# goldbricklemon/uplift-upsample-3dhpe

Hardware: AMD Instinct MI355X
Metric: pose-sequences/sec (higher is better)
Workload: dtype f16x3 (f32 operands split into f16 hi/lo, 3 MFMA passes, f32 accumulate); 1 GPU; config/h36m_351.json forward, N=71 tokens (receptive field 351), J=17, batch 128/GPU, s_in=5, seeded Keras-default weights; global_batch=128, parallelism=batch-sharded x1, hipgraph=True, concurrent_half_batches=False, batches_in_flight=8

## Files before the change

uplift-upsample-3dhpe_amd/csrc/uu3d_tchain16.h:

```cpp
#pragma once
#include <algorithm>
#include "uu3d_gemm_panel8.h"

namespace uu3d {

enum : int {
    TC_PROJ = 1,
    TC_MLP = 2,
    TC_QKV = 4,
    TC_FC1_PLANES = 8,
    TC_PE = 16,
};

static constexpr int TC_CHUNK_HALFS = P8_CHUNK_BYTES / 2;
__host__ __device__ inline constexpr int tchain_chunks(int flags) {
    return ((flags & TC_PROJ) ? 12 : 0) + ((flags & TC_MLP) ? 48 : 0) + ((flags & TC_FC1_PLANES) ? 24 : 0) + ((flags & TC_QKV) ? 36 : 0);
}
static constexpr size_t TC_TRASH_BYTES = 16384;

enum : int { TCP_BP = 0, TCP_B1 = 384, TCP_B2 = 1152, TCP_BQKV = 1536, TCP_FLOATS = 2688 };

struct TChainArgs {
    int M, m_tiles, period; float qscale;
    const _Float16* Of;
    float* X;
    float* XA; const float* pe;
    const _Float16* W;
    const float* P;
    _Float16* Q;
    _Float16* H;
    unsigned char* scratch;
};

__host__ __device__ inline size_t tchain_qf_index(size_t token, int ch, int plane) {
    const int u = ch >> 4, w = ch & 15, j = ((w >> 3) << 2) | (w & 3), g = (w >> 2) & 1;
    return ((((token >> 5) * 72 + u) * 2 + plane) * 64 + (token & 31) + 32 * g) * 8 + j;
}
__host__ __device__ inline constexpr size_t tchain_qf_halfs(int m_tiles) { return (size_t)m_tiles * 4 * 72 * 2 * 512; }

static constexpr size_t T16_X_FLOATS_PER_TILE = 64 * 384;
__host__ __device__ inline constexpr size_t tchain16_scratch_bytes(int m_tiles64) {
    return (size_t)m_tiles64 * (2 * T16_X_FLOATS_PER_TILE * 4) + TC_TRASH_BYTES;
}
inline void tchain16_reorder_mlp(const _Float16* in, _Float16* out) {
    const size_t C = TC_CHUNK_HALFS;
    std::copy(in, in + 12 * C, out);
    std::copy(in + 24 * C, in + 36 * C, out + 12 * C);
    std::copy(in + 12 * C, in + 24 * C, out + 24 * C);
    std::copy(in + 36 * C, in + 48 * C, out + 36 * C);
}

static constexpr size_t T16_XCHG_BYTES = 8 * 1024;
static constexpr size_t T16_BIAS_BYTES = 1152 * 4;
static constexpr size_t T16_LDS_TOTAL = P8_RING_BYTES + T16_XCHG_BYTES + T16_BIAS_BYTES;

__host__ __device__ inline size_t tchain16_xs_index(int row, int ch) {
    const int tile = row >> 6, q = (row >> 4) & 3, t = row & 15;
    const int c = ch >> 5, hh = (ch >> 4) & 1, g = (ch >> 2) & 3, r = ch & 3;
    return (size_t)tile * T16_X_FLOATS_PER_TILE + (((size_t)(c * 8 + 4 * hh + q) * 64 + t + 16 * g) * 4 + r);
}

inline void tchain16_pack_stage(const _Float16* Bh, const _Float16* Bl, int N, int Kp, int kofs, bool natural, _Float16* out) {
    for (int c = 0; c < N / 32; ++c)
        for (int hh = 0; hh < 2; ++hh)
            for (int kk = 0; kk < 12; ++kk)
                for (int p = 0; p < 2; ++p)
                    for (int l = 0; l < 64; ++l)
                        for (int j = 0; j < 8; ++j) {
                            const int S = kk >> 1, mm = kk & 1, t = l & 15, g = l >> 4;
                            const int n = 32 * c + 16 * (mm ^ hh) + t;
                            const int k = natural ? 16 * (12 * hh + 2 * S + (g >> 1)) + 8 * (j >> 2) + 4 * (g & 1) + (j & 3)
                                                  : kofs + 32 * (2 * S + (j >> 2)) + 16 * hh + 4 * g + (j & 3);
                            out[(((((size_t)c * 2 + hh) * 12 + kk) * 2 + p) * 64 + l) * 8 + j] = (p ? Bl : Bh)[(size_t)n * Kp + k];
                        }
}

template <bool BIAS> struct T16EpResidual { static constexpr int kStores = 0; static constexpr bool kBias = BIAS; const float* bias; int nbias; };
struct T16EpHidden { static constexpr int kStores = 0; static constexpr bool kBias = true; const float* bias; int nbias; };
struct T16EpQkv { static constexpr int kStores = 2; static constexpr bool kBias = true; h16x4* __restrict__ qf; const float* bias; int nbias; };
struct T16EpPlanes { static constexpr int kStores = 2; static constexpr bool kBias = true; unsigned char* __restrict__ ph; unsigned char* __restrict__ pl; const float* bias; int nbias; };

#ifndef UU3D_T16_DEPTH
#define UU3D_T16_DEPTH 2
#endif
#ifndef UU3D_T16_LOO
#define UU3D_T16_LOO 0
#endif

template <int FLAGS>
__global__ void __launch_bounds__(512) __attribute__((amdgpu_waves_per_eu(2, 2)))
tchain16_kernel(const TChainArgs a)
{
    constexpr int HS = 12, KS = 6;
    constexpr int GT = tchain_chunks(FLAGS);
    static_assert(!((FLAGS & TC_MLP) && (FLAGS & TC_FC1_PLANES)), "one MLP form per launch");
    static_assert(GT >= 12, "at least one stage");
    h3_flush_f16_denormals();
    extern __shared__ __attribute__((aligned(16))) unsigned char psm[];

    const int bm = blockIdx.x;
    const int tid = threadIdx.x, lane = tid & 63, wave = __builtin_amdgcn_readfirstlane(tid >> 6);
    const int hh = wave >> 2, q = wave & 3, g = lane >> 4, t = lane & 15;
    const int tok = bm * 64 + q * 16 + t;
    const bool live = tok < a.M;
    const int tokc = min(tok, a.M - 1);
    const int chl = 16 * hh + 4 * g;

    const unsigned wofs = (unsigned)(hh * HS * 2048 + q * 3072);
    const unsigned char* const wsrc = reinterpret_cast<const unsigned char*>(a.W) + wofs;
    const unsigned lane16 = (unsigned)lane * 16u;
    auto dma1 = [&](int Gc, int j, int slot, int i) __attribute__((always_inline)) {
        if (UU3D_T16_LOO & 1) return;
        const unsigned char* s = wsrc + (size_t)min(Gc, GT - 1) * P8_CHUNK_BYTES + j * (6 * 2048);
        unsigned char* d = psm + slot * P8_CHUNK_BYTES + wofs + j * (6 * 2048);
        switch (i) {
            case 0: __builtin_amdgcn_global_load_lds((h3_glb_void*)(s + lane16), (h3_lds_void*)d, 16, 0, 0); break;
            case 1: __builtin_amdgcn_global_load_lds((h3_glb_void*)(s + lane16), (h3_lds_void*)d, 16, 1024, 0); break;
            default: __builtin_amdgcn_global_load_lds((h3_glb_void*)(s + lane16), (h3_lds_void*)d, 16, 2048, 0); break;
        }
    };

    f32x4 xr[12];
    h16x8 ah[KS], al[KS];
    h16x8 fh[KS], fl[KS];
    constexpr int DP = UU3D_T16_DEPTH, RB = DP + 1;
    h16x8 bh[RB] = {}, bl[RB] = {};

    auto late = [&](int v) __attribute__((always_inline)) -> int { asm volatile("" : "+s"(v)); return v; };
    const unsigned xoff = (unsigned)(wave * 256 + lane * 4);
    auto xs_tile = [&](int b, bool strided1) __attribute__((always_inline)) -> float* {
        return reinterpret_cast<float*>(a.scratch) + ((size_t)b + (strided1 ? (size_t)a.m_tiles : 0)) * T16_X_FLOATS_PER_TILE;
    };
    auto load_xs = [&](const float* tl) __attribute__((always_inline)) {
#pragma unroll
        for (int c = 0; c < 12; ++c) xr[c] = *reinterpret_cast<const f32x4*>(tl + (xoff + (unsigned)(c * 2048)));
    };
    auto store_xs = [&](float* tl) __attribute__((always_inline)) {
        unsigned xo = xoff;
        asm volatile("" : "+v"(xo));
#pragma unroll
        for (int c = 0; c < 12; ++c) *reinterpret_cast<f32x4*>(tl + (xo + (unsigned)(c * 2048))) = xr[c];
    };
    auto load_rows = [&](const float* base) __attribute__((always_inline)) {
        const float* p = base + (size_t)tokc * 384 + chl;
#pragma unroll
        for (int c = 0; c < 12; ++c) xr[c] = *reinterpret_cast<const f32x4*>(p + 32 * c);
    };
    auto store_rows = [&](float* base) __attribute__((always_inline)) {
        const int tk = late(bm) * 64 + q * 16 + t;
        unsigned char* const tr = a.scratch + (size_t)a.m_tiles * (2 * T16_X_FLOATS_PER_TILE * 4);
        float* p = tk < a.M ? base + (size_t)tk * 384 + chl : reinterpret_cast<float*>(tr) + chl;
#pragma unroll
        for (int c = 0; c < 12; ++c) *reinterpret_cast<f32x4*>(p + 32 * c) = xr[c];
    };

    constexpr bool kStrided1 = (FLAGS & TC_FC1_PLANES) != 0;
    if constexpr ((FLAGS & TC_PROJ) != 0) {
        load_xs(xs_tile(bm, kStrided1));
        const int row0 = min(bm * 64 + q * 16, a.M - 1);
        const h16x8* ap = reinterpret_cast<const h16x8*>(a.Of) + (size_t)(row0 >> 5) * 24 * 2 * 64 + (row0 & 16) + t + 32 * (g & 1);
#pragma unroll
        for (int S = 0; S < KS; ++S) {
            const int sl = 12 * hh + 2 * S + (g >> 1);
            ah[S] = ap[(sl * 2 + 0) * 64]; al[S] = ap[(sl * 2 + 1) * 64];
        }
    } else {
        load_rows(a.X);
    }
#pragma unroll
    for (int g2 = 0; g2 < 5; ++g2)
#pragma unroll
        for (int i = 0; i < 3; ++i) dma1(g2 >> 1, g2 & 1, g2 >> 1, i);
    int G = 0, slot = 0;

    unsigned char* const xmine = psm + P8_RING_BYTES + wave * 1024 + lane16;
    unsigned char* const xpart = psm + P8_RING_BYTES + (wave ^ 4) * 1024 + lane16;
    float* const stat = reinterpret_cast<float*>(psm + P8_RING_BYTES);
    float* const bias_lds = reinterpret_cast<float*>(psm + P8_RING_BYTES + T16_XCHG_BYTES);
    const unsigned rd0 = (unsigned)(uintptr_t)(h3_lds_void*)(psm + hh * HS * 2048 + lane16);
    const unsigned bias_rd = (unsigned)(uintptr_t)(h3_lds_void*)(psm + P8_RING_BYTES + T16_XCHG_BYTES) + (unsigned)chl * 4u;

#define UU3D_T16_READ(i, sb, kk) \
    asm volatile("ds_read_b128 %0, %2 offset:%3\n\tds_read_b128 %1, %2 offset:%4" \
                 : "=&v"(bh[i]), "=&v"(bl[i]) : "v"(sb), "i"((kk) * 2048), "i"((kk) * 2048 + 1024))

    struct Acc { f32x4 a0[2], a1[2]; };
    struct Fin { f32x4 u, s, r, b, y; h16x4 vh, vl; };
    struct Keep { h16x4 h, l; };
    using I0 = std::integral_constant<int, 0>; using I1 = std::integral_constant<int, 1>; using I2 = std::integral_constant<int, 2>; using I3 = std::integral_constant<int, 3>;

    auto fin_a = [&](auto ep, auto fin_tag, const int j, Fin& f) __attribute__((always_inline)) {
        using EP = decltype(ep);
        constexpr int fs = decltype(fin_tag)::value;
        float y = f.u[j] + f.r[j];
        if constexpr (EP::kBias) y += f.b[j];
        if constexpr (std::is_same<EP, T16EpResidual<false>>::value || std::is_same<EP, T16EpResidual<true>>::value) {
            xr[fs][j] += y;
        } else {
            if constexpr (std::is_same<EP, T16EpHidden>::value || std::is_same<EP, T16EpPlanes>::value) y = fmaxf(y, 0.f);
            _Float16 h; float hf;
            asm("v_cvt_f16_f32 %0, %2\n\tv_cvt_f32_f16 %1, %0" : "=&v"(h), "=v"(hf) : "v"(y));
            f.y[j] = y - hf;
            f.vh[j] = h;
        }
    };
    auto fin_b = [&](auto ep, const int j, Fin& f) __attribute__((always_inline)) {
        using EP = decltype(ep);
        if constexpr (!(std::is_same<EP, T16EpResidual<false>>::value || std::is_same<EP, T16EpResidual<true>>::value))
            f.vl[j] = (_Float16)(f.y[j] * H3_SCALE);
    };
    auto fin_store = [&](auto ep, const int cp, auto fin_tag, Fin& f, Keep& hk) __attribute__((always_inline)) {
        using EP = decltype(ep);
        constexpr int fs = decltype(fin_tag)::value;
        if constexpr (std::is_same<EP, T16EpHidden>::value) {
            if constexpr ((fs & 1) == 0) { hk.h = f.vh; hk.l = f.vl; }
            else {
                h16x8 ph, pl;
#pragma unroll
                for (int e = 0; e < 4; ++e) { ph[e] = hk.h[e]; ph[4 + e] = f.vh[e]; pl[e] = hk.l[e]; pl[4 + e] = f.vl[e]; }
                constexpr int ks = fs == 11 ? 5 : fs >> 1;
                fh[ks] = ph; fl[ks] = pl;
            }
        } else if constexpr (std::is_same<EP, T16EpQkv>::value) {
            h16x4* d = ep.qf + (size_t)(2 * cp + hh) * 256;
            d[0] = f.vh; d[128] = f.vl;
        } else if constexpr (std::is_same<EP, T16EpPlanes>::value) {
            const unsigned o = (unsigned)(32 * cp) * 2u;
            *reinterpret_cast<h16x4*>(ep.ph + o) = f.vh;
            *reinterpret_cast<h16x4*>(ep.pl + o) = f.vl;
        }
    };

    auto chunk = [&](auto cl_tag, auto pre_tag, const int c, auto fin_tag, auto ep, const h16x8 (&Ah)[KS], const h16x8 (&Al)[KS],
                     Acc& x, const Acc& p, Keep& hk, const int bias_c0) __attribute__((always_inline)) {
        constexpr int CL = decltype(cl_tag)::value;
        constexpr bool PRE_IN = (decltype(pre_tag)::value & 1) != 0, PRE_OUT = (decltype(pre_tag)::value & 2) != 0;
        using EP = decltype(ep);
        constexpr int NST = EP::kStores;
        constexpr bool FIN = CL > 0 && !(UU3D_T16_LOO & 2);
        const int pslot = slot == 0 ? 2 : slot - 1;
        const unsigned sb = rd0 + (unsigned)slot * P8_CHUNK_BYTES;
        Fin f;
        auto gapwork = [&](const int gp) __attribute__((always_inline)) {
            if constexpr (CL > 0 && (UU3D_T16_LOO & 2) != 0) { if (gp == 3) asm volatile("" :: "v"(p.a0[0]), "v"(p.a0[1]), "v"(p.a1[0]), "v"(p.a1[1])); }
            if constexpr (FIN) {
                if (gp == 3 || gp == 4) {
#pragma unroll
                    for (int e = 0; e < 2; ++e) { const int k = 2 * (gp - 3) + e; f.s[k] = p.a0[1][k] + p.a1[1][k] * (1.0f / H3_SCALE); }
                }
                if (gp == 5) asm volatile("ds_write_b128 %0, %1" :: "v"((unsigned)(uintptr_t)(h3_lds_void*)xmine), "v"(f.s) : "memory");
                if (gp >= 9 && gp <= 12) f.u[gp - 9] = p.a0[0][gp - 9] + p.a1[0][gp - 9] * (1.0f / H3_SCALE);
                if (gp >= 22 && gp <= 25) fin_b(ep, gp - 22, f);
                if (gp >= 21 && gp <= 24) fin_a(ep, fin_tag, gp - 21, f);
                if (gp == 27) fin_store(ep, c - 1, fin_tag, f, hk);
            }
        };
        if constexpr (PRE_IN) asm volatile("s_waitcnt vmcnt(%0)" :: "i"(9 + NST * ((CL >= 2) + (CL >= 3))) : "memory");
        else asm volatile("s_waitcnt vmcnt(%0) lgkmcnt(0)" :: "i"(9 + NST * ((CL >= 2) + (CL >= 3))) : "memory");
        __builtin_amdgcn_sched_barrier(0);
        __builtin_amdgcn_s_barrier();
        __builtin_amdgcn_sched_barrier(0);
        if constexpr (!PRE_IN) {
#pragma unroll
            for (int d = 0; d < DP; ++d) UU3D_T16_READ(d, sb, d);
        }
#pragma unroll
        for (int m = 0; m < 2; ++m) { x.a0[m] = f32x4{0.f, 0.f, 0.f, 0.f}; x.a1[m] = f32x4{0.f, 0.f, 0.f, 0.f}; }
#define UU3D_T16_KK(kk) \
            x.a0[(kk) & 1] = __builtin_amdgcn_mfma_f32_16x16x32_f16(bh[(kk) % RB], Ah[(kk) >> 1], x.a0[(kk) & 1], 0, 0, 0); \
            __builtin_amdgcn_sched_barrier(0); gapwork(3 * (kk)); __builtin_amdgcn_sched_barrier(0); \
            x.a1[(kk) & 1] = __builtin_amdgcn_mfma_f32_16x16x32_f16(bh[(kk) % RB], Al[(kk) >> 1], x.a1[(kk) & 1], 0, 0, 0); \
            __builtin_amdgcn_sched_barrier(0); gapwork(3 * (kk) + 1); __builtin_amdgcn_sched_barrier(0); \
            x.a1[(kk) & 1] = __builtin_amdgcn_mfma_f32_16x16x32_f16(bl[(kk) % RB], Ah[(kk) >> 1], x.a1[(kk) & 1], 0, 0, 0); \
            __builtin_amdgcn_sched_barrier(0); gapwork(3 * (kk) + 2); __builtin_amdgcn_sched_barrier(0);
#pragma unroll
        for (int kk = 0; kk < 6; ++kk) {
            UU3D_T16_READ((kk + DP) % RB, sb, kk + DP);
            asm volatile("s_waitcnt lgkmcnt(%2)" : "+v"(bh[kk % RB]), "+v"(bl[kk % RB]) : "i"(2 * DP + (FIN && kk >= 2 && kk <= 1 + DP ? 1 : 0)));
            UU3D_T16_KK(kk)
            if ((kk & 1) == 0) dma1(G + 2, 1, pslot, kk >> 1);
            __builtin_amdgcn_sched_barrier(0);
        }
        asm volatile("s_waitcnt vmcnt(%0) lgkmcnt(%1)" :: "i"(9 + NST * (CL >= 2)), "i"(2 * DP) : "memory");
        __builtin_amdgcn_sched_barrier(0);
        __builtin_amdgcn_s_barrier();
        __builtin_amdgcn_sched_barrier(0);
        constexpr int NRB = FIN ? (EP::kBias ? 2 : 1) : 0;
        if constexpr (FIN) {
            asm volatile("ds_read_b128 %0, %1" : "=&v"(f.r) : "v"((unsigned)(uintptr_t)(h3_lds_void*)xpart) : "memory");
            if constexpr (EP::kBias) asm volatile("ds_read_b128 %0, %1" : "=&v"(f.b) : "v"(bias_rd + (unsigned)(bias_c0 + c - 1) * 128u) : "memory");
        }
#pragma unroll
        for (int kk = 6; kk < HS; ++kk) {
            if (kk + DP < HS) UU3D_T16_READ((kk + DP) % RB, sb, kk + DP);
            const int ahead = 2 * ((kk + DP < HS ? kk + DP : HS - 1) - kk);
            if (FIN && kk == 7) {
                const int behind = 6 + DP < HS ? 2 * ((7 + DP < HS ? 7 + DP : HS - 1) - (6 + DP) + 1) : 0;
                if constexpr (EP::kBias) asm volatile("s_waitcnt lgkmcnt(%4)" : "+v"(bh[kk % RB]), "+v"(bl[kk % RB]), "+v"(f.r), "+v"(f.b) : "i"(behind < ahead ? behind : ahead));
                else asm volatile("s_waitcnt lgkmcnt(%3)" : "+v"(bh[kk % RB]), "+v"(bl[kk % RB]), "+v"(f.r) : "i"(behind < ahead ? behind : ahead));
            }
            else asm volatile("s_waitcnt lgkmcnt(%2)" : "+v"(bh[kk % RB]), "+v"(bl[kk % RB]) : "i"(ahead + (FIN && kk == 6 ? NRB : 0)));
            UU3D_T16_KK(kk)
            if ((kk & 1) == 0) dma1(G + 3, 0, slot, (kk - 6) >> 1);
            __builtin_amdgcn_sched_barrier(0);
        }
#undef UU3D_T16_KK
        G += 1;
        slot = slot == 2 ? 0 : slot + 1;
        if constexpr (PRE_OUT) {
            const unsigned nb = rd0 + (unsigned)slot * P8_CHUNK_BYTES;
#pragma unroll
            for (int d = 0; d < DP; ++d) UU3D_T16_READ(d, nb, d);
        }
    };

    auto stage_tail = [&](auto ep, const int c, auto fin_tag, const Acc& p, Keep& hk, const int bias_c0) __attribute__((always_inline)) {
        using EP = decltype(ep);
        asm volatile("s_waitcnt vmcnt(0) lgkmcnt(0)" ::: "memory");
        __builtin_amdgcn_s_barrier();
        Fin f;
#pragma unroll
        for (int e = 0; e < 4; ++e) { f.s[e] = p.a0[1][e] + p.a1[1][e] * (1.0f / H3_SCALE); f.u[e] = p.a0[0][e] + p.a1[0][e] * (1.0f / H3_SCALE); }
        asm volatile("ds_write_b128 %0, %1\n\ts_waitcnt lgkmcnt(0)" :: "v"((unsigned)(uintptr_t)(h3_lds_void*)xmine), "v"(f.s) : "memory");
        __builtin_amdgcn_s_barrier();
        asm volatile("ds_read_b128 %0, %1" : "=&v"(f.r) : "v"((unsigned)(uintptr_t)(h3_lds_void*)xpart) : "memory");
        if constexpr (EP::kBias) asm volatile("ds_read_b128 %0, %1" : "=&v"(f.b) : "v"(bias_rd + (unsigned)(bias_c0 + c) * 128u) : "memory");
        else f.b = f32x4{0.f, 0.f, 0.f, 0.f};
        asm volatile("s_waitcnt lgkmcnt(0)" : "+v"(f.r), "+v"(f.b));
#pragma unroll
        for (int j = 0; j < 4; ++j) { fin_a(ep, fin_tag, j, f); fin_b(ep, j, f); }
        fin_store(ep, c, fin_tag, f, hk);
        __builtin_amdgcn_s_barrier();
    };

    using F0 = std::integral_constant<int, 0>; using F1 = std::integral_constant<int, 1>; using F2 = std::integral_constant<int, 2>; using F11 = std::integral_constant<int, 11>;
    auto stage = [&](auto nch_tag, auto ep, const h16x8 (&Ah)[KS], const h16x8 (&Al)[KS], const int bias_c0) __attribute__((always_inline)) {
        constexpr int NCH = decltype(nch_tag)::value;
        using EP = decltype(ep);
        static_assert(NCH % 4 == 0 && NCH >= 8, "bodies of four chunks");
        if constexpr (EP::kBias) {
            for (int i = tid; i < ep.nbias / 4; i += 512) reinterpret_cast<f32x4*>(bias_lds)[i] = reinterpret_cast<const f32x4*>(ep.bias)[i];
        }
        auto rotate = [&]() __attribute__((always_inline)) {
            if constexpr (std::is_same<EP, T16EpResidual<false>>::value || std::is_same<EP, T16EpResidual<true>>::value) {
                static_assert(NCH == 12, "three rotations");
#pragma unroll
                for (int s = 0; s < 4; ++s) { const f32x4 tt = xr[s]; xr[s] = xr[s + 4]; xr[s + 4] = xr[s + 8]; xr[s + 8] = tt; __builtin_amdgcn_sched_barrier(0); }
            } else if constexpr (std::is_same<EP, T16EpHidden>::value) {
                static_assert(NCH == 12, "three rotations");
#pragma unroll
                for (int s = 0; s < 2; ++s) {
                    const h16x8 th = fh[s], tl = fl[s];
                    fh[s] = fh[s + 2]; fl[s] = fl[s + 2]; fh[s + 2] = fh[s + 4]; fl[s + 2] = fl[s + 4]; fh[s + 4] = th; fl[s + 4] = tl;
                    __builtin_amdgcn_sched_barrier(0);
                }
            }
        };
        Acc xa, xb;
#pragma unroll
        for (int m = 0; m < 2; ++m) { xb.a0[m] = f32x4{0.f, 0.f, 0.f, 0.f}; xb.a1[m] = f32x4{0.f, 0.f, 0.f, 0.f}; }
        Keep hk{};
        chunk(I0{}, I2{}, 0, F0{}, ep, Ah, Al, xa, xb, hk, bias_c0);
        chunk(I1{}, I3{}, 1, F0{}, ep, Ah, Al, xb, xa, hk, bias_c0);
        chunk(I2{}, I3{}, 2, F1{}, ep, Ah, Al, xa, xb, hk, bias_c0);
        chunk(I3{}, I1{}, 3, F2{}, ep, Ah, Al, xb, xa, hk, bias_c0);
        rotate();
#pragma unroll 1
        for (int c = 4; c < NCH; c += 4) {
            chunk(I3{}, I2{}, c, F11{}, ep, Ah, Al, xa, xb, hk, bias_c0);
            chunk(I3{}, I3{}, c + 1, F0{}, ep, Ah, Al, xb, xa, hk, bias_c0);
            chunk(I3{}, I3{}, c + 2, F1{}, ep, Ah, Al, xa, xb, hk, bias_c0);
            chunk(I3{}, I1{}, c + 3, F2{}, ep, Ah, Al, xb, xa, hk, bias_c0);
            rotate();
        }
        stage_tail(ep, (int)(NCH - 1), F11{}, xb, hk, bias_c0);
    };
    using N12 = std::integral_constant<int, 12>;

    auto token_sum = [&](float s, int phase) __attribute__((always_inline)) -> float {
        s += __shfl_xor(s, 16);
        s += __shfl_xor(s, 32);
        if (g == 0) stat[phase * 128 + wave * 16 + t] = s;
        asm volatile("s_waitcnt lgkmcnt(0)" ::: "memory");
        __builtin_amdgcn_s_barrier();
        asm volatile("" ::: "memory");
        return s + stat[phase * 128 + (wave ^ 4) * 16 + t];
    };
    auto layer_norm = [&]() __attribute__((always_inline)) {
        float s = 0.f;
#pragma unroll
        for (int c = 0; c < 12; ++c) s += (xr[c][0] + xr[c][1]) + (xr[c][2] + xr[c][3]);
        const float mean = token_sum(s, 0) * (1.0f / 384.0f);
        float v = 0.f;
#pragma unroll
        for (int c = 0; c < 12; ++c) {
            const f32x4 d = xr[c] - mean;
            v += (d[0] * d[0] + d[1] * d[1]) + (d[2] * d[2] + d[3] * d[3]);
        }
        const float rstd = 1.0f / sqrtf(token_sum(v, 1) * (1.0f / 384.0f) + 1e-5f);
#pragma unroll
        for (int S = 0; S < KS; ++S) {
            h16x4 hi[2], lo[2];
#pragma unroll
            for (int i = 0; i < 2; ++i) h3_split((xr[2 * S + i] - mean) * rstd, hi[i], lo[i]);
#pragma unroll
            for (int e = 0; e < 4; ++e) { ah[S][e] = hi[0][e]; ah[S][4 + e] = hi[1][e]; al[S][e] = lo[0][e]; al[S][4 + e] = lo[1][e]; }
        }
    };

    if constexpr ((FLAGS & TC_PROJ) != 0) {
        stage(N12{}, T16EpResidual<true>{a.P + TCP_BP, 384}, ah, al, 0);
        if constexpr (kStrided1) store_rows(a.XA);
    } else {
        store_xs(xs_tile(bm, false));
    }
    if constexpr ((FLAGS & (TC_MLP | TC_FC1_PLANES)) != 0) {
        layer_norm();
        if constexpr (kStrided1) {
            unsigned char* const trash = a.scratch + (size_t)a.m_tiles * (2 * T16_X_FLOATS_PER_TILE * 4);
            unsigned char* ph = live ? reinterpret_cast<unsigned char*>(a.H + (size_t)tok * 768 + chl) : trash;
            unsigned char* pl = live ? reinterpret_cast<unsigned char*>(a.H + ((size_t)a.M + tok) * 768 + chl) : trash + 4096;
            stage(std::integral_constant<int, 24>{}, T16EpPlanes{ph, pl, a.P + TCP_B1, 768}, ah, al, 0);
        } else {
            stage(N12{}, T16EpHidden{a.P + TCP_B1, 384}, ah, al, 0);
            stage(N12{}, T16EpResidual<false>{nullptr, 0}, fh, fl, 0);
            stage(N12{}, T16EpHidden{a.P + TCP_B1 + 384, 384}, ah, al, 0);
            stage(N12{}, T16EpResidual<true>{a.P + TCP_B2, 384}, fh, fl, 0);
            if constexpr ((FLAGS & TC_QKV) == 0 || (FLAGS & TC_PE) != 0) store_rows(a.X);
        }
    }
    if constexpr ((FLAGS & TC_QKV) != 0) {
        if constexpr ((FLAGS & TC_PE) != 0) {
            const int tkc = min(late(bm) * 64 + q * 16 + t, a.M - 1);
            const float* pr = a.pe + (size_t)(tkc % a.period) * 384 + chl;
#pragma unroll
            for (int c = 0; c < 12; ++c) xr[c] = xr[c] + *reinterpret_cast<const f32x4*>(pr + 32 * c);
            store_xs(xs_tile(late(bm), true));
        } else if constexpr ((FLAGS & (TC_PROJ | TC_MLP)) != 0) {
            store_xs(xs_tile(late(bm), false));
        }
        layer_norm();
        const int lb = late(bm);
        h16x4* const qf = reinterpret_cast<h16x4*>(a.Q) + ((size_t)(lb * 2 + (q >> 1)) * (72 * 2 * 64) + (q & 1) * 16 + t + 32 * (g & 1)) * 2 + (g >> 1);
        stage(std::integral_constant<int, 36>{}, T16EpQkv{qf, a.P + TCP_BQKV, 1152}, ah, al, 0);
    }
    asm volatile("s_waitcnt vmcnt(0)" ::: "memory");
#undef UU3D_T16_READ
}

}
```

Before: 209,900 pose-sequences/s.

## Seed accumulators with bias and pack f16 hi/lo split conversions

The bias is no longer read and added in the epilogue. It is loaded from LDS straight into the first accumulator before the MFMA chain, so it rides along in the GEMM accumulation. The f16 hi/lo split now uses packed v_cvt_pk_f16_f32 and v_fma_mix instructions, handling two values per step and storing them as packed u32 pairs. This cuts VALU work and an LDS read in the epilogue gaps, at the cost of more intricate lgkmcnt bookkeeping and an extra LDS load placed before the chunk reads.

```diff
diff --git a/uplift-upsample-3dhpe_amd/csrc/uu3d_tchain16.h b/uplift-upsample-3dhpe_amd/csrc/uu3d_tchain16.h
--- a/uplift-upsample-3dhpe_amd/csrc/uu3d_tchain16.h
+++ b/uplift-upsample-3dhpe_amd/csrc/uu3d_tchain16.h
@@ -184,30 +184,40 @@
     asm volatile("ds_read_b128 %0, %2 offset:%3\n\tds_read_b128 %1, %2 offset:%4" \
                  : "=&v"(bh[i]), "=&v"(bl[i]) : "v"(sb), "i"((kk) * 2048), "i"((kk) * 2048 + 1024))
 
+    typedef unsigned u32x2 __attribute__((ext_vector_type(2)));
+    typedef unsigned u32x4 __attribute__((ext_vector_type(4)));
     struct Acc { f32x4 a0[2], a1[2]; };
-    struct Fin { f32x4 u, s, r, b, y; h16x4 vh, vl; };
-    struct Keep { h16x4 h, l; };
+    struct Fin { f32x4 u, s, r, y; u32x2 vh, vl; };
+    struct Keep { u32x2 h, l; };
     using I0 = std::integral_constant<int, 0>; using I1 = std::integral_constant<int, 1>; using I2 = std::integral_constant<int, 2>; using I3 = std::integral_constant<int, 3>;
 
+    const float split_scale = H3_SCALE;
     auto fin_a = [&](auto ep, auto fin_tag, const int j, Fin& f) __attribute__((always_inline)) {
         using EP = decltype(ep);
         constexpr int fs = decltype(fin_tag)::value;
-        float y = f.u[j] + f.r[j];
-        if constexpr (EP::kBias) y += f.b[j];
         if constexpr (std::is_same<EP, T16EpResidual<false>>::value || std::is_same<EP, T16EpResidual<true>>::value) {
-            xr[fs][j] += y;
+            xr[fs][j] += f.u[j] + f.r[j];
         } else {
-            if constexpr (std::is_same<EP, T16EpHidden>::value || std::is_same<EP, T16EpPlanes>::value) y = fmaxf(y, 0.f);
-            _Float16 h; float hf;
-            asm("v_cvt_f16_f32 %0, %2\n\tv_cvt_f32_f16 %1, %0" : "=&v"(h), "=v"(hf) : "v"(y));
-            f.y[j] = y - hf;
+            if (j >= 2) return;
+            float y0 = f.u[2 * j] + f.r[2 * j], y1 = f.u[2 * j + 1] + f.r[2 * j + 1];
+            if constexpr (std::is_same<EP, T16EpHidden>::value || std::is_same<EP, T16EpPlanes>::value) { y0 = fmaxf(y0, 0.f); y1 = fmaxf(y1, 0.f); }
+            unsigned h;
+            asm("v_cvt_pk_f16_f32 %0, %1, %2" : "=v"(h) : "v"(y0), "v"(y1));
+            f.y[2 * j] = y0; f.y[2 * j + 1] = y1;
             f.vh[j] = h;
         }
     };
     auto fin_b = [&](auto ep, const int j, Fin& f) __attribute__((always_inline)) {
         using EP = decltype(ep);
-        if constexpr (!(std::is_same<EP, T16EpResidual<false>>::value || std::is_same<EP, T16EpResidual<true>>::value))
-            f.vl[j] = (_Float16)(f.y[j] * H3_SCALE);
+        if constexpr (!(std::is_same<EP, T16EpResidual<false>>::value || std::is_same<EP, T16EpResidual<true>>::value)) {
+            if (j >= 2) return;
+            float d0, d1; unsigned l;
+            asm("v_fma_mix_f32 %0, %1, 1.0, -%2 op_sel_hi:[0,0,1]" : "=v"(d0) : "v"(f.y[2 * j]), "v"(f.vh[j]));
+            asm("v_fma_mix_f32 %0, %1, 1.0, -%2 op_sel:[0,0,1] op_sel_hi:[0,0,1]" : "=v"(d1) : "v"(f.y[2 * j + 1]), "v"(f.vh[j]));
+            asm("v_fma_mixlo_f16 %0, %1, %2, 0 op_sel_hi:[0,0,0]" : "=v"(l) : "v"(d0), "s"(split_scale));
+            asm("v_fma_mixhi_f16 %0, %1, %2, 0 op_sel_hi:[0,0,0]" : "+v"(l) : "v"(d1), "s"(split_scale));
+            f.vl[j] = l;
+        }
     };
     auto fin_store = [&](auto ep, const int cp, auto fin_tag, Fin& f, Keep& hk) __attribute__((always_inline)) {
         using EP = decltype(ep);
@@ -215,29 +225,28 @@
         if constexpr (std::is_same<EP, T16EpHidden>::value) {
             if constexpr ((fs & 1) == 0) { hk.h = f.vh; hk.l = f.vl; }
             else {
-                h16x8 ph, pl;
-#pragma unroll
-                for (int e = 0; e < 4; ++e) { ph[e] = hk.h[e]; ph[4 + e] = f.vh[e]; pl[e] = hk.l[e]; pl[4 + e] = f.vl[e]; }
                 constexpr int ks = fs == 11 ? 5 : fs >> 1;
-                fh[ks] = ph; fl[ks] = pl;
+                fh[ks] = __builtin_bit_cast(h16x8, u32x4{hk.h[0], hk.h[1], f.vh[0], f.vh[1]});
+                fl[ks] = __builtin_bit_cast(h16x8, u32x4{hk.l[0], hk.l[1], f.vl[0], f.vl[1]});
             }
         } else if constexpr (std::is_same<EP, T16EpQkv>::value) {
             h16x4* d = ep.qf + (size_t)(2 * cp + hh) * 256;
-            d[0] = f.vh; d[128] = f.vl;
+            d[0] = __builtin_bit_cast(h16x4, f.vh); d[128] = __builtin_bit_cast(h16x4, f.vl);
         } else if constexpr (std::is_same<EP, T16EpPlanes>::value) {
             const unsigned o = (unsigned)(32 * cp) * 2u;
-            *reinterpret_cast<h16x4*>(ep.ph + o) = f.vh;
-            *reinterpret_cast<h16x4*>(ep.pl + o) = f.vl;
+            *reinterpret_cast<u32x2*>(ep.ph + o) = f.vh;
+            *reinterpret_cast<u32x2*>(ep.pl + o) = f.vl;
         }
     };
 
     auto chunk = [&](auto cl_tag, auto pre_tag, const int c, auto fin_tag, auto ep, const h16x8 (&Ah)[KS], const h16x8 (&Al)[KS],
-                     Acc& x, const Acc& p, Keep& hk, const int bias_c0) __attribute__((always_inline)) {
+                     Acc& x, Acc& p, Keep& hk, const int bias_c0) __attribute__((always_inline)) {
         constexpr int CL = decltype(cl_tag)::value;
         constexpr bool PRE_IN = (decltype(pre_tag)::value & 1) != 0, PRE_OUT = (decltype(pre_tag)::value & 2) != 0;
         using EP = decltype(ep);
         constexpr int NST = EP::kStores;
         constexpr bool FIN = CL > 0 && !(UU3D_T16_LOO & 2);
+        constexpr bool SEED = EP::kBias && !(UU3D_T16_LOO & 2);
         const int pslot = slot == 0 ? 2 : slot - 1;
         const unsigned sb = rd0 + (unsigned)slot * P8_CHUNK_BYTES;
         Fin f;
@@ -250,8 +259,12 @@
                 }
                 if (gp == 5) asm volatile("ds_write_b128 %0, %1" :: "v"((unsigned)(uintptr_t)(h3_lds_void*)xmine), "v"(f.s) : "memory");
                 if (gp >= 9 && gp <= 12) f.u[gp - 9] = p.a0[0][gp - 9] + p.a1[0][gp - 9] * (1.0f / H3_SCALE);
-                if (gp >= 22 && gp <= 25) fin_b(ep, gp - 22, f);
-                if (gp >= 21 && gp <= 24) fin_a(ep, fin_tag, gp - 21, f);
+                if constexpr (std::is_same<EP, T16EpResidual<false>>::value || std::is_same<EP, T16EpResidual<true>>::value) {
+                    if (gp >= 21 && gp <= 24) fin_a(ep, fin_tag, gp - 21, f);
+                } else {
+                    if (gp == 21 || gp == 23) fin_a(ep, fin_tag, (gp - 21) >> 1, f);
+                    if (gp == 22 || gp == 24) fin_b(ep, (gp - 22) >> 1, f);
+                }
                 if (gp == 27) fin_store(ep, c - 1, fin_tag, f, hk);
             }
         };
@@ -261,11 +274,12 @@
         __builtin_amdgcn_s_barrier();
         __builtin_amdgcn_sched_barrier(0);
         if constexpr (!PRE_IN) {
+            if constexpr (SEED) asm volatile("ds_read_b128 %0, %1" : "=&v"(x.a0[0]) : "v"(bias_rd + (unsigned)(bias_c0 + c) * 128u) : "memory");
 #pragma unroll
             for (int d = 0; d < DP; ++d) UU3D_T16_READ(d, sb, d);
         }
-#pragma unroll
-        for (int m = 0; m < 2; ++m) { x.a0[m] = f32x4{0.f, 0.f, 0.f, 0.f}; x.a1[m] = f32x4{0.f, 0.f, 0.f, 0.f}; }
+        if constexpr (!SEED) x.a0[0] = f32x4{0.f, 0.f, 0.f, 0.f};
+        x.a0[1] = f32x4{0.f, 0.f, 0.f, 0.f}; x.a1[0] = f32x4{0.f, 0.f, 0.f, 0.f}; x.a1[1] = f32x4{0.f, 0.f, 0.f, 0.f};
 #define UU3D_T16_KK(kk) \
             x.a0[(kk) & 1] = __builtin_amdgcn_mfma_f32_16x16x32_f16(bh[(kk) % RB], Ah[(kk) >> 1], x.a0[(kk) & 1], 0, 0, 0); \
             __builtin_amdgcn_sched_barrier(0); gapwork(3 * (kk)); __builtin_amdgcn_sched_barrier(0); \
@@ -276,7 +290,8 @@
 #pragma unroll
         for (int kk = 0; kk < 6; ++kk) {
             UU3D_T16_READ((kk + DP) % RB, sb, kk + DP);
-            asm volatile("s_waitcnt lgkmcnt(%2)" : "+v"(bh[kk % RB]), "+v"(bl[kk % RB]) : "i"(2 * DP + (FIN && kk >= 2 && kk <= 1 + DP ? 1 : 0)));
+            if (SEED && kk == 0) asm volatile("s_waitcnt lgkmcnt(%3)" : "+v"(bh[0]), "+v"(bl[0]), "+v"(x.a0[0]) : "i"(2 * DP));
+            else asm volatile("s_waitcnt lgkmcnt(%2)" : "+v"(bh[kk % RB]), "+v"(bl[kk % RB]) : "i"(2 * DP + (FIN && kk >= 2 && kk <= 1 + DP ? 1 : 0)));
             UU3D_T16_KK(kk)
             if ((kk & 1) == 0) dma1(G + 2, 1, pslot, kk >> 1);
             __builtin_amdgcn_sched_barrier(0);
@@ -285,19 +300,15 @@
         __builtin_amdgcn_sched_barrier(0);
         __builtin_amdgcn_s_barrier();
         __builtin_amdgcn_sched_barrier(0);
-        constexpr int NRB = FIN ? (EP::kBias ? 2 : 1) : 0;
-        if constexpr (FIN) {
-            asm volatile("ds_read_b128 %0, %1" : "=&v"(f.r) : "v"((unsigned)(uintptr_t)(h3_lds_void*)xpart) : "memory");
-            if constexpr (EP::kBias) asm volatile("ds_read_b128 %0, %1" : "=&v"(f.b) : "v"(bias_rd + (unsigned)(bias_c0 + c - 1) * 128u) : "memory");
-        }
+        constexpr int NRB = FIN ? 1 : 0;
+        if constexpr (FIN) asm volatile("ds_read_b128 %0, %1" : "=&v"(f.r) : "v"((unsigned)(uintptr_t)(h3_lds_void*)xpart) : "memory");
 #pragma unroll
         for (int kk = 6; kk < HS; ++kk) {
             if (kk + DP < HS) UU3D_T16_READ((kk + DP) % RB, sb, kk + DP);
             const int ahead = 2 * ((kk + DP < HS ? kk + DP : HS - 1) - kk);
             if (FIN && kk == 7) {
                 const int behind = 6 + DP < HS ? 2 * ((7 + DP < HS ? 7 + DP : HS - 1) - (6 + DP) + 1) : 0;
-                if constexpr (EP::kBias) asm volatile("s_waitcnt lgkmcnt(%4)" : "+v"(bh[kk % RB]), "+v"(bl[kk % RB]), "+v"(f.r), "+v"(f.b) : "i"(behind < ahead ? behind : ahead));
-                else asm volatile("s_waitcnt lgkmcnt(%3)" : "+v"(bh[kk % RB]), "+v"(bl[kk % RB]), "+v"(f.r) : "i"(behind < ahead ? behind : ahead));
+                asm volatile("s_waitcnt lgkmcnt(%3)" : "+v"(bh[kk % RB]), "+v"(bl[kk % RB]), "+v"(f.r) : "i"(behind < ahead ? behind : ahead));
             }
             else asm volatile("s_waitcnt lgkmcnt(%2)" : "+v"(bh[kk % RB]), "+v"(bl[kk % RB]) : "i"(ahead + (FIN && kk == 6 ? NRB : 0)));
             UU3D_T16_KK(kk)
@@ -309,12 +320,13 @@
         slot = slot == 2 ? 0 : slot + 1;
         if constexpr (PRE_OUT) {
             const unsigned nb = rd0 + (unsigned)slot * P8_CHUNK_BYTES;
+            if constexpr (SEED) asm volatile("ds_read_b128 %0, %1" : "=&v"(p.a0[0]) : "v"(bias_rd + (unsigned)(bias_c0 + c + 1) * 128u) : "memory");
 #pragma unroll
             for (int d = 0; d < DP; ++d) UU3D_T16_READ(d, nb, d);
         }
     };
 
-    auto stage_tail = [&](auto ep, const int c, auto fin_tag, const Acc& p, Keep& hk, const int bias_c0) __attribute__((always_inline)) {
+    auto stage_tail = [&](auto ep, const int c, auto fin_tag, const Acc& p, Keep& hk) __attribute__((always_inline)) {
         using EP = decltype(ep);
         asm volatile("s_waitcnt vmcnt(0) lgkmcnt(0)" ::: "memory");
         __builtin_amdgcn_s_barrier();
@@ -324,9 +336,7 @@
         asm volatile("ds_write_b128 %0, %1\n\ts_waitcnt lgkmcnt(0)" :: "v"((unsigned)(uintptr_t)(h3_lds_void*)xmine), "v"(f.s) : "memory");
         __builtin_amdgcn_s_barrier();
         asm volatile("ds_read_b128 %0, %1" : "=&v"(f.r) : "v"((unsigned)(uintptr_t)(h3_lds_void*)xpart) : "memory");
-        if constexpr (EP::kBias) asm volatile("ds_read_b128 %0, %1" : "=&v"(f.b) : "v"(bias_rd + (unsigned)(bias_c0 + c) * 128u) : "memory");
-        else f.b = f32x4{0.f, 0.f, 0.f, 0.f};
-        asm volatile("s_waitcnt lgkmcnt(0)" : "+v"(f.r), "+v"(f.b));
+        asm volatile("s_waitcnt lgkmcnt(0)" : "+v"(f.r));
 #pragma unroll
         for (int j = 0; j < 4; ++j) { fin_a(ep, fin_tag, j, f); fin_b(ep, j, f); }
         fin_store(ep, c, fin_tag, f, hk);
@@ -373,7 +383,7 @@
             chunk(I3{}, I1{}, c + 3, F2{}, ep, Ah, Al, xb, xa, hk, bias_c0);
             rotate();
         }
-        stage_tail(ep, (int)(NCH - 1), F11{}, xb, hk, bias_c0);
+        stage_tail(ep, (int)(NCH - 1), F11{}, xb, hk);
     };
     using N12 = std::integral_constant<int, 12>;
 
```

Result: no change. 210,400 pose-sequences/s, median of 5 (+0.2%).
